# alv-around/mini-stark

Measured on AMD Instinct MI355X. Metric: stark_proofs_per_s, higher is better.
Workload: dtype u64; 1 GPU; Fibonacci AIR, Goldilocks, 2^20 trace rows, blowup 8, 20 security bits (w=3, c=6, rounds=23, ood_queries=1, fri_queries=2); a step = 8 independent proofs in flight per GPU

## Files before the change

### mini-stark_amd/csrc/ctx.hpp

```cpp
#pragma once
#include "../../include/ministark.h"

#include <cstdarg>
#include <cstdio>
#include <cstdlib>
#include <map>
#include <new>
#include <string>
#include <type_traits>
#include <vector>

#include "field.hpp"
#include "merkle.hpp"
#include "ntt.hpp"
#include "poly.hpp"

namespace msctx {

struct DevBuf {
  void* p = nullptr; size_t cap = 0;
  int ensure(size_t bytes) {
    if (bytes <= cap) return 0;
    if (p) msrt::free_dev(p);
    p = nullptr; cap = 0;
// ... 165 lines not shown
    launched();
    if (gx == 0 || gy == 0) return 0;
    if (!prof_on) return msrt::launch_coop<K>(stream, gx, gy, threads, lds, p);
    ProfRec r; r.kid = kid; r.sub = next_sub; r.bytes = next_bytes; r.part = part_depth > 0; next_bytes = 0; next_sub = 0;
    if (msrt::event_create(&r.a) || msrt::event_create(&r.b)) return 1;
    msrt::event_record(r.a, stream);
    int e = msrt::launch_coop<K>(stream, gx, gy, threads, lds, p);
    msrt::event_record(r.b, stream);
    prof_recs.push_back(r);
    return e;
  }
  template <class K> int run(int kid, unsigned gx, unsigned gy, int threads, size_t lds, const typename K::Params& p) {
    launched();
    if (gx == 0 || gy == 0) return 0;
    if (!prof_on) return msrt::launch<K>(stream, gx, gy, threads, lds, p);
    ProfRec r; r.kid = kid; r.sub = next_sub; r.bytes = next_bytes; r.part = part_depth > 0; next_bytes = 0; next_sub = 0;
    if (msrt::event_create(&r.a) || msrt::event_create(&r.b)) return 1;
    msrt::event_record(r.a, stream);
    int e = msrt::launch<K>(stream, gx, gy, threads, lds, p);
    msrt::event_record(r.b, stream);
    prof_recs.push_back(r);
    return e;
  }
  int profile_begin() override { prof_on = true; return 0; }
  int profile_end(char* out, size_t cap) override;

  struct Plan {
    int log_n = 0, log_r0 = 0, log_rho = 0, npass = 0, K[4] = {0, 0, 0, 0}, lo_bits = 0;
    int LC[4] = {msntt::TILE_LOG_C, msntt::TILE_LOG_C, msntt::TILE_LOG_C, msntt::TILE_LOG_C};
    bool v2[4] = {false, false, false, false};
    bool regp[4] = {false, false, false, false};
    DevBuf tw_lo, tw_hi, w_r[4], vtw, w0;
    T n_inv = 0;
  };
  std::map<int, Plan*> plans;
  DevBuf ntt_scratch;
  int ntt_kmax = 9;
  int ntt_v2 = 1, ntt_v2_regpass = 1;
  int ntt_fast = 1;

  int get_plan(int log_n, int log_pad, bool inverse, Plan** out);

  template <bool INV, int K, int TH>
  int launch_fast(const msntt::PassParams<F>& pp, size_t tiles, size_t batch);
  template <class KK> int launch_v2i(const msntt::PassParams<F>& pp, unsigned grid, int nsub, int mode, int k, int lc);
  template <bool INV, int K, int LC, int MODE>
  int launch_v2m(const msntt::PassParams<F>& pp, size_t tiles, size_t batch);
  int ntt_coop_wgs = 512, ntt_share = 1;
  unsigned coop_grid(size_t work_items, int per_cu = 2) const { const size_t g = (size_t)ntt_coop_wgs * per_cu / 2; return (unsigned)(work_items < g ? work_items : g); }
  template <bool INV, int K, int LC>
  int launch_v2(const msntt::PassParams<F>& pp, size_t tiles, size_t batch);
  template <bool INV, int LC>
  int launch_v2k(const msntt::PassParams<F>& pp, size_t tiles, size_t batch);
  template <bool INV, int K>
  int launch_reg(const msntt::PassParams<F>& pp, size_t batch);
  template <bool INV>
  int launch_pass(const msntt::PassParams<F>& pp, size_t tiles, size_t batch, bool v2 = false, bool regp = false);

  int ntt_run(int log_n, bool inverse, const T* src, size_t src_bstride, size_t n_in, T* dst, size_t dst_bstride, size_t batch);
  int scale_pow(const T* src, size_t src_bstride, T* dst, size_t dst_bstride, size_t n, T s, size_t batch);

  void* h_tabs = nullptr; size_t h_tabs_cap = 0;
  int tabs_host(size_t bytes, u8** out);
  DevBuf d_zero; size_t zero_used = 0, zero_cap = 0;
  int zero_alloc(size_t bytes, void** out);

// ... 4 lines not shown
                size_t g_first = 0, u32 run_len = 0, u32 run_stride = 0, const msmerkle::LinColSpec* lin = nullptr, size_t out_g0 = 0);
  template <int EL>
  int tree_build(const T* base, size_t col_stride, size_t row_stride, size_t limb_stride, u32 width, const TreeShape& ts, DevBuf& nodes, const msmerkle::LinColSpec* lin = nullptr);
  u32* host_root() const { return reinterpret_cast<u32*>(reinterpret_cast<u8*>(pinned) + 256); }
  bool root_on_host = false;
  unsigned long long* pending_aux = nullptr; bool aux_on_host = false;
  int inner_levels(u32* nodes, size_t nchildren, size_t ic, bool final_levels = true, u8* rec_out = nullptr);
  int inner_launch(unsigned grid, const msmerkle::InnerHashParams& ip);
  template <int EL>
  int tree_build_sharded(const T* base, size_t col_stride, size_t row_stride, size_t limb_stride, u32 width, TreeShape& ts, DevBuf& nodes, const msmerkle::LinColSpec* lin = nullptr);
  unsigned long long* shard_aux = nullptr;
  int finish_sharded_tree(TreeShape& ts, DevBuf& nodes, size_t Mloc);
  template <int EL>
  int tree_build_sharded_contiguous(const T* base, size_t col_stride, size_t row_stride, size_t limb_stride, u32 width, TreeShape& ts, DevBuf& nodes);
  int read_root(const DevBuf& nodes, const TreeShape& ts, u8* root);

  size_t N = 0, w = 0, L = 0, blowup = 0;
  int npolys = 0; size_t polys_cap = 0;
  struct Lin { std::vector<u64> s; std::vector<int> idx; };
  std::vector<Lin> poly_lin;
  std::vector<char> poly_mat; int lazy_lin = 1;
  void expand(int i, T scale, std::map<int, T>& acc) const {
    const Lin& li = poly_lin[i];
    if (li.idx.empty()) { auto it = acc.find(i); if (it == acc.end()) acc[i] = scale; else it->second = F::add(it->second, scale); return; }
    for (size_t t = 0; t < li.idx.size(); t++) expand(li.idx[t], F::mul(scale, F::from_u64(li.s[t] % F::P)), acc);
  }
  int materialize(int i);
  bool have_trace = false, have_polys = false, have_lde = false, have_validity = false;
  DevBuf d_trace[2], d_polys, d_coef, d_lde, d_trace_nodes, d_lde_nodes, d_io, d_partials, d_small;
  TreeShape trace_ts, lde_ts;
  size_t lde_c = 0;

  struct Round { DevBuf poly, cw, nodes; size_t cap = 0, ncoef = 0, D = 0; TreeShape ts; size_t m = 0;
                 bool dist = false, local_store = false; size_t S = 0; };
  size_t shard_gather_chunk = 0;
  int shard_dist = 1;
  int proof_root_only = 0;
  const T* lpoly(const Round* r) const { return r->local_store ? r->poly.template as<T>() : r->poly.template as<T>() + (size_t)sh_rank * r->S; }
  size_t lstride(const Round* r) const { return r->local_store ? r->S : r->cap; }
  size_t lcount(const Round* r, size_t n) const { const size_t lo = (size_t)sh_rank * r->S; return n <= lo ? 0 : (n - lo < r->S ? n - lo : r->S); }
  size_t dist_chunk(size_t D) const {
    if (!sh_on || !shard_dist || !fri_blowup || !shardable(D / 2)) return 0;
    const size_t den = fri_blowup * (size_t)sh_world;
    if (D % den) return 0;
    const size_t S = D / den;
    return (S >= 2 && !(S & 1)) ? S : 0;
  }
  DevBuf d_carry, d_lq, d_pack, d_fullpoly;
  std::vector<Round*> rounds; size_t nrounds_done = 0, fri_rounds = 0, fri_blowup = 0;
  bool have_deep = false; XE cur_z; XE cur_B[2];
  DevBuf d_folded, d_sh, d_blob, d_tabs, d_targets, d_idx, d_deg, d_ovf;
  size_t blob_size = 0;

  int ensure_polys(size_t count);

  int init(int dev, u32 flags);
  ~Ctx() {
    for (auto& kv : plans) { kv.second->tw_lo.release(); kv.second->tw_hi.release(); kv.second->vtw.release(); kv.second->w0.release(); for (auto& b : kv.second->w_r) b.release(); delete kv.second; }
    drop_rccl();
    if (sdma_pending) msrt::Sdma::get().wait(sdma_sig, -1.0);
    else if (copy_pending) msrt::event_sync(ev_copy);
    if (up.pending) msrt::Sdma::get().wait(sdma_up_sig, -1.0);
    if (sdma_state == 1) { msrt::Sdma::get().signal_destroy(sdma_sig); msrt::Sdma::get().signal_destroy(sdma_up_sig); }
    for (msrt::Event* e : ev_hash) msrt::event_destroy(e);
    for (msrt::Event* e : ev_xchg) msrt::event_destroy(e);
    if (comm_stream) msrt::stream_destroy(comm_stream);
    if (side_stream) { msrt::sync(side_stream); msrt::stream_destroy(side_stream); }
// ... 154 lines not shown
```

### mini-stark_amd/csrc/field.hpp

```cpp
#pragma once
#include "rt.hpp"

typedef uint64_t u64;
typedef uint32_t u32;
typedef uint8_t u8;

struct GL {
  typedef u64 T;
  static constexpr int ID = 0;
  static constexpr u64 P = 0xFFFFFFFF00000001ULL;
  static constexpr u64 EPS = 0xFFFFFFFFULL;
  static constexpr u64 GENERATOR = 7;
  static constexpr int TWO_ADICITY = 32;
  static constexpr int EXT = 2;
  static constexpr u64 NR2 = 7;
  static constexpr int MAX_DIGITS = 20;
  static MS_HD u32 hi(u64 x) { return (u32)(x >> 32); }
  static MS_HD u32 lo(u64 x) { return (u32)x; }
  static MS_HD u64 mk(u32 l, u32 h) { return ((u64)h << 32) | l; }
  static MS_HD T add(T a, T b) {
    const T s = a + b;
    const T t = s - P;
    return (s < a || s >= P) ? t : s;
  }
  static MS_HD T sub(T a, T b) {
    T d = a - b;
    if (a < b) d -= EPS;
    return d;
  }
  static MS_HD T neg(T a) { return a ? P - a : 0; }
  static MS_HD T reduce128(u64 lo_, u64 hi_) {
    const u64 hi_hi = hi_ >> 32, hi_lo = hi_ & EPS;
    u64 t0 = lo_ - hi_hi;
    t0 -= (lo_ < hi_hi) ? EPS : 0;
    const u64 t1 = (hi_lo << 32) - hi_lo;
    const u64 r = t0 + t1;
    const u64 r2 = r + EPS;
    return (r < t1 || r >= P) ? r2 : r;
  }
  static MS_HD T mul(T a, T b) {
    const u32 a0 = (u32)a, a1 = (u32)(a >> 32), b0 = (u32)b, b1 = (u32)(b >> 32);
    const u64 p00 = (u64)a0 * b0;
    const u64 p01 = (u64)a0 * b1 + (p00 >> 32);
    const u64 p10 = (u64)a1 * b0 + (u32)p01;
    const u64 p11 = (u64)a1 * b1 + (p01 >> 32) + (p10 >> 32);
    return reduce128((p10 << 32) | (u32)p00, p11);
  }
  static MS_HD T from_u64(u64 v) { return v; }
  static MS_HD u64 to_u64(T v) { return v; }
  static MS_HD T to_tw(T w) { return w; }
  static MS_HD T tw_of(T w) { return w; }
  static MS_HD T mul_tw(T a, T w_tab) { return mul(a, w_tab); }
  static MS_HD T from_tw(T w_tab) { return w_tab; }
};

struct GLT : GL {
  static MS_HD u64 sel(u32 m, u64 t, u64 s) { return mk(ms_bitop3<0xCA>(m, lo(t), lo(s)), ms_bitop3<0xCA>(m, hi(t), hi(s))); }
  static MS_HD T add(T a, T b) {
    const u64 s = a + b, t = s + EPS;
    const u32 c1 = ms_bitop3<0xD4>(hi(a), hi(b), hi(s));
    const u32 m = ms_sar31(ms_bitop3<0xF4>(c1, hi(s), hi(t)));
    return sel(m, t, s);
  }
  static MS_HD T sub(T a, T b) {
    const u64 d = a - b;
    const u32 bo = ms_bitop3<0x8E>(hi(a), hi(b), hi(d));
    return d + ms_pin64(mk(bo >> 31, ms_sar31(bo)));
  }
  static MS_HD T fold_small(u64 A, u32 h) {
    const u64 r = (u64)h * 0xFFFFFFFFu + A, t = r + EPS;
    return sel(ms_sar31(ms_bitop3<0x74>(hi(A), hi(r), hi(t))), t, r);
  }
  static MS_HD T reduce128(u64 lo_, u64 hi_) {
    const u32 h0 = lo(hi_), h1 = hi(hi_);
    const u64 A = lo_ - h1;
    const u32 b1 = ms_bitop3<0x0C>(hi(lo_), hi(A), 0u);
    const u64 U = (u64)h0 * 0xFFFFFFFFu;
    const u64 r = A + U, t = r + EPS;
    const u32 c1 = ms_bitop3<0xD4>(hi(A), hi(U), hi(r));
    const u32 c2 = ms_bitop3<0x30>(hi(r), hi(t), 0u);
// ... 267 lines not shown
```

### mini-stark_amd/csrc/fri_commit.cpp

```cpp
#include "ctx.hpp"
#include "fri_tail.hpp"

namespace msctx {

template <class F>
int Ctx<F>::round_commit(Round* r, size_t ncoef_in, int nonzero_limbs, const Round* prev, const XE* alpha) {
  if (ctz64(r->D) > F::TWO_ADICITY) return fail(MS_ERR_SHAPE, "FRI domain larger than the field's two-adicity");
  RQ(tree_shape(r->D, 2, 2, &r->ts));
  r->m = 0;
  {
    const bool shard_next = shardable(r->D / 2);
    bool z_outside_base = false;
    for (int l = 1; l < E; l++) z_outside_base = z_outside_base || cur_z.c[l] != 0;
    if (prev && fri_pointwise && z_outside_base && prev->D == 2 * r->D && prev->ts.sharded == shard_next) {
      Plan* pl;
      RQ(get_plan(ctz64(prev->D), 0, false, &pl));
      const size_t W = (size_t)sh_world;
      const size_t m_out = shard_next ? r->D / (2 * W) : r->D;
      const size_t local = shard_next ? 2 * m_out : r->D;
      if (shard_next) r->m = m_out;
      if (r->cw.ensure(local * E * sizeof(T))) return fail(MS_ERR_NOMEM, "codeword");
      const size_t total = m_out * (shard_next ? 2 : 1);
      const XE c = e_add<F, E>(cur_B[0], e_mul<F>(cur_B[1], *alpha));
      auto fold_launch = [&](auto* kernel) {
        typedef typename std::remove_pointer<decltype(kernel)>::type FK;
        typename FK::Params fp;
        fp.src = prev->cw.template as<T>(); fp.src_limb_stride = shard_next ? 2 * prev->m : prev->D;
        fp.dst = r->cw.template as<T>(); fp.dst_limb_stride = local;
        fp.m_out = m_out; fp.log_m = (u32)ctz64(m_out); fp.groups = shard_next ? 2 : 1; fp.shard_W = shard_next ? (u32)W : 0; fp.shard_k = (u32)sh_rank;
        fp.tw_lo = pl->tw_lo.template as<T>(); fp.tw_hi = pl->tw_hi.template as<T>(); fp.lo_bits = (u32)pl->lo_bits; fp.log_D = (u32)ctz64(prev->D);
        fp.alpha = *alpha;
        fp.c2 = e_add<F, E>(c, c);
        fp.z = cur_z;
        fp.inv2 = f_inv<F>(F::from_u64(2));
        return run<FK>(K_FOLD, grid1(total, FK::THREADS * FK::ITEMS), 1, FK::THREADS, 0, fp);
      };
      next_bytes = (double)total * E * sizeof(T) * 3;
      { PartScopeIf part(this, shard_next); CK(total <= fold_small_max ? fold_launch((mspoly::FriFoldEvalKernel<F, E, 1>*)nullptr) : fold_launch((mspoly::FriFoldEvalKernel<F, E, 8>*)nullptr)); }
      if (shard_next) RQ((tree_build_sharded<E>(r->cw.template as<T>(), m_out, 1, 2 * m_out, 2, r->ts, r->nodes)));
      else RQ((tree_build<E>(r->cw.template as<T>(), 0, 1, r->D, 1, r->ts, r->nodes)));
      return 0;
    }
  }
  RQ(join_side());
  if (shardable(r->D / 2)) {
    const size_t m = r->D / (2 * (size_t)sh_world);
    r->m = m;
    if (r->cw.ensure(2 * m * E * sizeof(T))) return fail(MS_ERR_NOMEM, "codeword");
    const T* coef = r->poly.template as<T>(); size_t coef_stride = r->cap;
    if (r->local_store) {
      const size_t full = r->S * (size_t)sh_world;
      if (d_fullpoly.ensure(full * E * sizeof(T))) return fail(MS_ERR_NOMEM, "gathered polynomial");
      if (ncoef_in) RQ(gather_poly(lpoly(r), r->S, ncoef_in, d_fullpoly.as<T>(), full));
      coef = d_fullpoly.as<T>(); coef_stride = full;
    }
    { PartScope part(this); RQ(coset_eval(coef, coef_stride, ncoef_in, ctz64(r->D), F::from_u64(1), 2, r->cw.template as<T>(), 2 * m, (size_t)nonzero_limbs)); }
    if (nonzero_limbs < E) CK(msrt::memset_dev(r->cw.template as<T>() + (size_t)nonzero_limbs * 2 * m, 0, (size_t)(E - nonzero_limbs) * 2 * m * sizeof(T), stream));
    RQ((tree_build_sharded<E>(r->cw.template as<T>(), m, 1, 2 * m, 2, r->ts, r->nodes)));
    return 0;
  }
  if (r->cw.ensure(r->D * E * sizeof(T))) return fail(MS_ERR_NOMEM, "codeword");
  RQ(ntt_run(ctz64(r->D), false, r->poly.template as<T>(), r->cap, ncoef_in, r->cw.template as<T>(), r->D, (size_t)nonzero_limbs));
  if (nonzero_limbs < E) CK(msrt::memset_dev(r->cw.template as<T>() + (size_t)nonzero_limbs * r->D, 0, (size_t)(E - nonzero_limbs) * r->D * sizeof(T), stream));
  RQ((tree_build<E>(r->cw.template as<T>(), 0, 1, r->D, 1, r->ts, r->nodes)));
  return 0;
}

template <class F>
int Ctx<F>::degree_launch(const T* poly, size_t limb_stride, size_t n, unsigned long long** dres_out) {
  void* zr;
  RQ(zero_alloc(8, &zr));
  unsigned long long* dres = reinterpret_cast<unsigned long long*>(zr);
  if (n) {
    typename mspoly::DegreeKernel<F, E>::Params dp{poly, limb_stride, n, dres, 0};
    CK(run<mspoly::DegreeKernel<F, E>>(K_DEGREE, grid1(n, mspoly::THREADS), 1, mspoly::THREADS, 0, dp));
  }
  *dres_out = dres;
  return 0;
}

template <class F>
int Ctx<F>::read_degree_and_root(const T* poly, size_t limb_stride, size_t n, Round* r, size_t* ncoef, u8* root) {
  unsigned long long* dres = nullptr;
  RQ(degree_launch(poly, limb_stride, n, &dres));
  const bool on_host = r && root_on_host;
  CK(msrt::d2h(pinned, dres, 8, stream));
  if (r && !on_host) CK(msrt::d2h(reinterpret_cast<u8*>(pinned) + 64, r->nodes.template as<u8>() + (r->ts.local_nodes - 1) * 32, 32, stream));
  CK(msrt::sync(stream));
  *ncoef = (size_t)(*reinterpret_cast<unsigned long long*>(pinned));
  if (r && root) memcpy(root, on_host ? reinterpret_cast<const u8*>(host_root()) : reinterpret_cast<const u8*>(pinned) + 64, 32);
  return 0;
}

template <class F>
int Ctx<F>::fri_begin(size_t blowup_, size_t nrounds, u8* root0) {
  if (!have_validity) return fail(MS_ERR_STATE, "fri_begin before mix");
// ... 170 lines not shown
    CK(run<CKn>(K_SUFFIX_HORNER, 1, 1, CKn::THREADS, 0, cp));
    if (mj) for (int l = pl.nl - 1; l >= 0; l--) RQ(sh_launch_inline(pl.fin[l], 1));
    nq_coef = m - 1;
  }
  nr->S = Sn;
  if (next_dist) { nr->dist = true; nr->local_store = true; }
  else {
    if (nr->poly.ensure(nr->cap * E * sizeof(T))) return fail(MS_ERR_NOMEM, "fold");
    if (nq_coef) RQ(gather_poly(lq, Sn, nq_coef, nr->poly.template as<T>(), nr->cap));
    nr->S = 0;
  }
  *nq_coef_out = nq_coef;
  return 0;
}

template <class F>
int Ctx<F>::fri_tail_round(Round* pr, Round* nr, const XE& a, bool* done) {
  if (digest == MS_DIGEST_KECCAK256) return fri_tail_round_t<msmerkle::Keccak256Kernels>(pr, nr, a, done);
  if (digest == MS_DIGEST_SHA3_256) return fri_tail_round_t<msmerkle::Sha3_256Kernels>(pr, nr, a, done);
  if (digest == MS_DIGEST_BLAKE3) return fri_tail_round_t<msmerkle::Blake3Kernels>(pr, nr, a, done);
  return digest == MS_DIGEST_BLAKE2S256 ? fri_tail_round_t<msmerkle::Blake2sKernels>(pr, nr, a, done) : fri_tail_round_t<msmerkle::Sha256Kernels>(pr, nr, a, done);
}
template <class F> template <class DG>
int Ctx<F>::fri_tail_round_t(Round* pr, Round* nr, const XE& a, bool* done) {
  *done = false;
  const size_t n = pr->ncoef, m = (n + 1) / 2, Dn = nr->D, M = Dn / 2;
  bool z_outside_base = false;
  for (int l = 1; l < E; l++) z_outside_base = z_outside_base || cur_z.c[l] != 0;
  if (!fri_tail_max || pr->D > fri_tail_max || pr->dist || pr->ts.sharded || shardable(M) || !fri_pointwise || !z_outside_base || m > (size_t)mspoly::SH_BS || M < 1) return 0;
  typedef msfri::FriTailKernel<F, E, DG> TK;
  if (M > (size_t)TK::WG_GROUPS << TK::TreeK::MAX_LEVELS) return 0;
  if (ctz64(Dn) > F::TWO_ADICITY) return fail(MS_ERR_SHAPE, "FRI domain larger than the field's two-adicity");
  RQ(tree_shape(Dn, 2, 2, &nr->ts));
  nr->m = 0;
  if (nr->poly.ensure(nr->cap * E * sizeof(T)) || d_folded.ensure((m + 1) * E * sizeof(T)) || nr->cw.ensure(Dn * E * sizeof(T)) || nr->nodes.ensure(nr->ts.nodes * 32) ||
      d_sh.ensure(sh_scratch_elems(m) * sizeof(T)))
    return fail(MS_ERR_NOMEM, "fused FRI round");
  Plan* pl;
  RQ(get_plan(ctz64(pr->D), 0, false, &pl));
  typename TK::Params tp;
  memset(&tp, 0, sizeof tp);
  tp.do_coef = m >= 2 ? 1 : 0;
  tp.fold = typename TK::FoldK::Params{pr->poly.template as<T>(), pr->cap, n, d_folded.as<T>(), m, a, nullptr};
  if (tp.do_coef) {
    SHPlan sp = sh_plan(d_folded.as<T>(), m, 0, 1, m, cur_z, nr->poly.template as<T>(), false, nr->cap, 0, 1, nullptr, d_sh.as<T>());
    if (sp.nl != 1) return fail(MS_ERR_STATE, "fused FRI round: scan of more than one block");
    tp.scan.jobs = nullptr; tp.scan.inline_job = sp.fin[0]; tp.scan.final_mode = 1;
  }
  unsigned long long* dres = d_deg.as<unsigned long long>();
  tp.deg = typename TK::DegK::Params{nr->poly.template as<T>(), nr->cap, m >= 2 ? m - 1 : 0, dres, 0};
  const size_t per = M < (size_t)TK::WG_GROUPS ? M : (size_t)TK::WG_GROUPS, G = M / per;
  tp.G = (u32)G;
  const XE c = e_add<F, E>(cur_B[0], e_mul<F>(cur_B[1], a));
  tp.eval.src = pr->cw.template as<T>(); tp.eval.src_limb_stride = pr->D; tp.eval.dst = nr->cw.template as<T>(); tp.eval.dst_limb_stride = Dn;
  tp.eval.m_out = Dn; tp.eval.log_m = (u32)ctz64(Dn); tp.eval.groups = 1; tp.eval.shard_W = 0; tp.eval.shard_k = 0;
  tp.eval.tw_lo = pl->tw_lo.template as<T>(); tp.eval.tw_hi = pl->tw_hi.template as<T>(); tp.eval.lo_bits = (u32)pl->lo_bits; tp.eval.log_D = (u32)ctz64(pr->D);
  tp.eval.alpha = a; tp.eval.c2 = e_add<F, E>(c, c); tp.eval.z = cur_z; tp.eval.inv2 = f_inv<F>(F::from_u64(2));
  tp.leaf.base = nr->cw.template as<T>(); tp.leaf.col_stride = 0; tp.leaf.row_stride = 1; tp.leaf.limb_stride = Dn; tp.leaf.width = 1; tp.leaf.lpn = 2;
  tp.leaf.zero_as_empty = zae; tp.leaf.ngroups = M; tp.leaf.nodes = nr->nodes.template as<u32>();
  u32 nl = 0; while (((size_t)1 << nl) < per) nl++;
  tp.sub.nodes = nr->nodes.template as<u32>(); tp.sub.child_off = 0; tp.sub.nchildren = M; tp.sub.ic = 2; tp.sub.nlevels = nl;
  u32 tl = 0; while (((size_t)1 << tl) < G) tl++;
  tp.top.nodes = nr->nodes.template as<u32>(); tp.top.child_off = 2 * M - 2 * G; tp.top.nchildren = G; tp.top.ic = 2; tp.top.nlevels = tl;
  tp.top.host_root = host_root(); tp.top.aux_src = dres; tp.top.aux_dst = reinterpret_cast<unsigned long long*>(pinned); tp.top.flag = arm_flag();
  tp.root_index = nr->ts.nodes - 1;
  tp.done = reinterpret_cast<u32*>(d_deg.as<u8>() + 128);
  next_bytes = (double)Dn * E * sizeof(T) * 3 + (double)M * 96;
// ... 115 lines not shown
```

### mini-stark_amd/csrc/ntt_plan.cpp

```cpp
#include "ctx.hpp"

namespace msctx {

template <class F>
int Ctx<F>::get_plan(int log_n, int log_pad, bool inverse, Plan** out) {
  int key = (log_n * 4 + log_pad) * 2 + (inverse ? 1 : 0);
  auto it = plans.find(key);
  if (it != plans.end()) { *out = it->second; return 0; }
  if (log_n > F::TWO_ADICITY) return fail(MS_ERR_SHAPE, "domain larger than the field's two-adicity");
  Plan* pl = new Plan();
  pl->log_n = log_n;
  const int v2_lc = (F::ID == 0) ? 3 : 4;
  bool use_v2 = false;
  if (ntt_v2 >= 1 && log_n >= 14 && log_n > msntt::MAX_LOG_R && (log_pad == 0 || log_pad == 3)) {
    const int m = log_n - log_pad, P = (m + 9) / 10;
    const int kb = (ntt_v2_regpass == 2) ? 7 : 10;
    if (ntt_v2_regpass && m - 2 * kb >= 1 && m - 2 * kb <= 5) {
      use_v2 = true;
      pl->log_rho = 0; pl->log_r0 = log_pad; pl->npass = 3;
      pl->K[0] = kb; pl->K[1] = kb; pl->K[2] = m - 2 * kb;
      pl->LC[0] = log_pad ? 3 : v2_lc; pl->LC[1] = v2_lc; pl->LC[2] = 0;
      pl->v2[0] = pl->v2[1] = true; pl->regp[2] = true;
    } else if (P <= 2 && m / P >= 7) {
      use_v2 = true;
      pl->log_rho = 0; pl->log_r0 = log_pad; pl->npass = P;
      for (int i = 0; i < P; i++) {
        pl->K[i] = m / P + (i < m % P ? 1 : 0); pl->LC[i] = (i == 0 && log_pad) ? 3 : v2_lc; pl->v2[i] = true;
      }
    }
  }
  if (use_v2) {}
  else if (log_n <= msntt::MAX_LOG_R) { pl->npass = 1; pl->K[0] = log_n; }
  else {
    int best_rho = 0, bestP = 1 << 20;
    for (int lr = 0; lr <= (log_pad ? msntt::MAX_LOG_RHO : 0); lr++) {
      const int m = log_n - log_pad - lr;
      if (m < 2) break;
      int P = (m + ntt_kmax - 1) / ntt_kmax;
      if (P < 2 && log_pad == 0) P = 2;
      if (P < 1) P = 1;
      if (P < bestP) { bestP = P; best_rho = lr; }
    }
    if (ntt_fast && bestP > 1 && (log_pad == 0 || (log_n >= 22 && log_n <= 24))) {
      best_rho = 0; log_pad = 0;
      bestP = (log_n + ntt_kmax - 1) / ntt_kmax; if (bestP < 2) bestP = 2;
    }
    pl->log_rho = best_rho; pl->log_r0 = log_pad + best_rho;
    const int m = log_n - pl->log_r0, P = bestP;
    pl->npass = P;
    for (int i = 0; i < P; i++) pl->K[i] = m / P + (i < m % P ? 1 : 0);
  }
  const int log_r0 = pl->log_r0;
  T wn = f_root_of_unity<F>(log_n);
  if (inverse) wn = f_inv<F>(wn);
  const size_t n = (size_t)1 << log_n;
  pl->n_inv = f_inv<F>(F::from_u64(n % F::P));
  pl->lo_bits = (log_n + 1) / 2;
  const size_t nlo = (size_t)1 << pl->lo_bits, nhi = (size_t)1 << (log_n - pl->lo_bits);
  std::vector<T> lo(nlo), hi(nhi);
  T x = F::from_u64(1);
  for (size_t j = 0; j < nlo; j++) { lo[j] = F::to_tw(x); x = F::mul(x, wn); }
  T wh = x;
  x = F::from_u64(1);
  for (size_t j = 0; j < nhi; j++) { hi[j] = F::to_tw(x); x = F::mul(x, wh); }
  if (pl->tw_lo.ensure(nlo * sizeof(T)) || pl->tw_hi.ensure(nhi * sizeof(T))) { delete pl; return fail(MS_ERR_NOMEM, "twiddle tables"); }
  CK(msrt::h2d(pl->tw_lo.p, lo.data(), nlo * sizeof(T), stream));
  CK(msrt::h2d(pl->tw_hi.p, hi.data(), nhi * sizeof(T), stream));
  CK(msrt::sync(stream));
  for (int i = 0; i < pl->npass; i++) {
    const size_t r = (size_t)1 << pl->K[i];
    T wr = f_root_of_unity<F>(pl->K[i]);
    if (inverse) wr = f_inv<F>(wr);
    std::vector<T> tab(r);
    x = F::from_u64(1);
    for (size_t j = 0; j < r; j++) { tab[j] = F::to_tw(x); x = F::mul(x, wr); }
    if (pl->w_r[i].ensure(r * sizeof(T))) { delete pl; return fail(MS_ERR_NOMEM, "w_r table"); }
    CK(msrt::h2d(pl->w_r[i].p, tab.data(), r * sizeof(T), stream));
    CK(msrt::sync(stream));
  }
  if (pl->log_r0) {
    const size_t cnt = (size_t)1 << log_r0;
    T wv = f_root_of_unity<F>(log_r0);
    if (inverse) wv = f_inv<F>(wv);
    std::vector<T> tab(cnt);
    x = F::from_u64(1);
    for (size_t j = 0; j < cnt; j++) { tab[j] = F::to_tw(x); x = F::mul(x, wv); }
    if (pl->w0.ensure(cnt * sizeof(T))) { delete pl; return fail(MS_ERR_NOMEM, "w0 table"); }
// ... 247 lines not shown
```

### mini-stark_amd/csrc/poly.hpp

```cpp
#pragma once
#include "field.hpp"
#include "ntt.hpp"

namespace mspoly {

constexpr int THREADS = 256;

template <class F> struct TransposeInKernel {
  typedef typename F::T T;
  static constexpr int THREADS = mspoly::THREADS;
  struct Params { const u64* src; T* dst; size_t N, w, dst_stride; T rinv; int mont;  u32* bad; };
  static MS_HD int nphases(const Params&) { return 1; }
  static MS_DEV void phase(int, const Params& p, int bx, int, int tid, int nthreads, unsigned char*) {
    const size_t f = (size_t)bx * nthreads + tid;
    if (f >= p.N * p.w) return;
    const size_t row = f / p.w, col = f - row * p.w;
    const u64 raw = p.src[f];
    const bool oob = raw >= F::P;
    if (oob && p.bad) *p.bad = 1;
    T v = F::from_u64(oob ? 0 : raw);
    if (p.mont) v = F::mul(v, p.rinv);
    p.dst[col * p.dst_stride + row] = v;
  }
};
// ... 439 lines not shown
        const size_t ia = t * 2 * p.m_out + i, ib = ia + p.m_out;
        const size_t r = p.shard_W ? 2 * ((size_t)p.shard_k + (size_t)p.shard_W * i) + t : i;
        X a, b;
#pragma unroll
        for (int l = 0; l < E; l++) { a.c[l] = p.src[(size_t)l * p.src_limb_stride + ia]; b.c[l] = p.src[(size_t)l * p.src_limb_stride + ib]; }
        const X s = e_add<F, E>(a, b), d = e_sub<F, E>(a, b);
        const T xinv = w_tab(p, (Dm + 1 - r) & Dm);
        X u;
#pragma unroll
        for (int l = 0; l < E; l++) u.c[l] = F::mul_tw(p.alpha.c[l], xinv);
        const X num = e_sub<F, E>(e_add<F, E>(s, e_mul<F>(u, d)), p.c2);
        const T y = F::from_tw(w_tab(p, (2 * r) & Dm));
        X C;
        inv_parts(p, F::sub(y, p.z.c[0]), &C, &nrm[it]);
        tt[it] = e_mul<F>(num, C);
      }
      pre[it] = run;
      run = F::mul(run, nrm[it]);
    }
    T inv = F::mul(fold_base_inv<F>(run), p.inv2);
#pragma unroll
    for (int it = ITEMS - 1; it >= 0; it--) {
      const size_t j = j0 + (size_t)it * nthreads;
      const T ni = F::mul(inv, pre[it]);
      inv = F::mul(inv, nrm[it]);
      if (j < total) {
#pragma unroll
        for (int l = 0; l < E; l++) p.dst[(size_t)l * p.dst_limb_stride + j] = F::mul(tt[it].c[l], ni);
      }
    }
  }
};

template <class F, int E> struct DegreeKernel {
  typedef typename F::T T;
  static constexpr int THREADS = mspoly::THREADS;
  struct Params { const T* src; size_t limb_stride, n; unsigned long long* result; size_t idx0; };
  static MS_HD int nphases(const Params&) { return 1; }
  static MS_DEV void phase(int, const Params& p, int bx, int, int tid, int nthreads, unsigned char*) {
    const size_t r = (size_t)bx * nthreads + tid;
    if (r >= p.n) return;
    const size_t j = p.n - 1 - r;
    if ((unsigned long long)(p.idx0 + j + 1) <= *reinterpret_cast<volatile unsigned long long*>(p.result)) return;
    bool nz = false, nz_next = false;
    for (int l = 0; l < E; l++) nz = nz || (p.src[(size_t)l * p.limb_stride + j] != 0);
    if (nz && j + 1 < p.n) for (int l = 0; l < E; l++) nz_next = nz_next || (p.src[(size_t)l * p.limb_stride + j + 1] != 0);
    if (nz && !nz_next) msrt::atomic_max_u64(p.result, (unsigned long long)(p.idx0 + j + 1));
  }
};
template <class F, int E> struct FindJob {
  const typename F::T* src; size_t limb_stride, n;
  const typename F::T* targets ; int nt; unsigned long long* result;
  u32 map_g, map_W, map_k; size_t map_m;
};
template <class F, int E> struct FindFirstKernel {
  typedef typename F::T T;
  static constexpr int THREADS = mspoly::THREADS;
  struct Params { const FindJob<F, E>* jobs; FindJob<F, E> inline_job; };
  static MS_HD int nphases(const Params&) { return 1; }
  static MS_DEV void phase(int, const Params& pp, int bx, int by, int tid, int nthreads, unsigned char*) {
    const FindJob<F, E>& p = pp.jobs ? pp.jobs[by] : pp.inline_job;
    const size_t j = (size_t)bx * nthreads + tid;
    if (j >= p.n) return;
    T v[E];
    for (int l = 0; l < E; l++) v[l] = p.src[(size_t)l * p.limb_stride + j];
    for (int t = 0; t < p.nt; t++) {
// ... 177 lines not shown
      const T root = p.ex_roots[k];
#pragma unroll
      for (int it = 0; it < ITEMS; it++) acc[it] = F::mul(acc[it], F::sub(x[it], root));
    }
#pragma unroll
    for (int it = 0; it < ITEMS; it++) {
      const size_t i = i0 + (size_t)it * THREADS;
      if (i < p.L) p.out[i] = F::mul(acc[it], p.den_inv[i & (size_t)(p.blowup - 1)]);
    }
  }
};

template <int S> struct ArithShift { template <class A> static MS_DEV u64 run(u64 x, int s) { return s == S ? msntt::gl_mul_pow2<S, A>(x) : ArithShift<S - 1>::template run<A>(x, s); } };
template <> struct ArithShift<0> { template <class A> static MS_DEV u64 run(u64 x, int) { return x; } };
template <class F, class A> struct ArithKernel {
  typedef typename F::T T;
  static constexpr int THREADS = 256;
  struct Params { const u64* a; const u64* b; u64* out; size_t n; int op; };
  static MS_HD int nphases(const Params&) { return 1; }
  static MS_DEV void phase(int, const Params& p, int bx, int, int tid, int, unsigned char*) {
    const size_t i = (size_t)bx * THREADS + tid;
    if (i >= p.n) return;
    const T a = F::from_u64(p.a[i]), b = F::from_u64(p.b[i]);
    T r = 0;
    if (p.op == 0) r = A::add(a, b);
    else if (p.op == 1) r = A::sub(a, b);
    else if (p.op == 2) r = A::mul(a, b);
    else if (p.op == 3) r = A::mul_tw(a, F::to_tw(b));
    if constexpr (F::ID == 0) {
      if (p.op == 4) r = A::mul_x32(a);
      else if (p.op == 5) r = A::mul_x64(a);
      else if (p.op == 6) r = ArithShift<95>::template run<A>(a, (int)(p.b[i] % 96));
      else if (p.op == 7) r = A::fold_small(a, (u32)p.b[i] & 0x7FFFFFFFu);
    }
    p.out[i] = F::to_u64(r);
  }
};
}
```

### mini-stark_amd/csrc/session.cpp

```cpp
#include "ctx.hpp"

namespace msctx {

template <class F>
int Ctx<F>::profile_end(char* out, size_t cap) {
  static const char* names[K_COUNT] = {"ntt_pass", "scale_pow", "leaf_hash", "inner_hash", "transpose_in", "io_copy", "lincomb", "mix", "eval", "eval_reduce",
                                       "fold", "suffix_horner", "degree", "find_first", "merkle_path", "query_points", "fri_tail", "mix_terms"};
  msrt::sync(stream);
  double ms[K_COUNT] = {0}, by[K_COUNT] = {0}, ms_part = 0, ms_repl = 0, repl_by[K_COUNT] = {0}; unsigned long long cnt[K_COUNT] = {0};
  std::map<int, double> sub_ms, sub_by; std::map<int, unsigned long long> sub_cnt;
  for (auto& r : prof_recs) {
    float t = 0.f; msrt::event_elapsed_ms(&t, r.a, r.b);
    ms[r.kid] += t; by[r.kid] += r.bytes; cnt[r.kid]++;
    if (r.part) ms_part += t; else { ms_repl += t; repl_by[r.kid] += t; }
    if (r.kid == K_NTT_PASS) { sub_ms[r.sub] += t; sub_by[r.sub] += r.bytes; sub_cnt[r.sub]++; }
    msrt::event_destroy(r.a); msrt::event_destroy(r.b);
  }
  prof_recs.clear(); prof_on = false;
  std::string j = "{";
  for (int k = 0; k < K_COUNT; k++) {
    char buf[256];
    snprintf(buf, sizeof buf, "%s\"%s\": {\"launches\": %llu, \"ms\": %.6f, \"alg_bytes\": %.0f}", k ? ", " : "", names[k], cnt[k], ms[k], by[k]);
    j += buf;
  }
// ... 189 lines not shown
  for (int t = 0; t < k; t++) if (idx[t] < 0 || idx[t] >= npolys || s[t] >= F::P) return fail(MS_ERR_ARG, "lincomb index/scalar out of range");
  RQ(ensure_polys(npolys + 2));
  if (!lazy_lin) RQ(lincomb_into(d_polys.as<T>(), N, N, s, idx, k, npolys, d_polys.as<T>() + (size_t)npolys * N));
  poly_mat.push_back(lazy_lin ? 0 : 1);
  { Lin l; l.s.assign(s, s + k); l.idx.assign(idx, idx + k); poly_lin.push_back(l); }
  npolys++; have_lde = have_validity = false;
  return MS_OK;
}

template <class F>
int Ctx<F>::polys_append(const u64* coeffs, size_t n) {
  if (!have_polys) return fail(MS_ERR_STATE, "append before interpolate");
  if (!coeffs || n > N) return fail(MS_ERR_SHAPE, "constraint polynomial has more than N coefficients (starks.rs:118-119 asserts)");
  if (!canonical(coeffs, n)) return fail(MS_ERR_ARG, "coefficient not canonical");
  RQ(ensure_polys(npolys + 2));
  T* dst = d_polys.as<T>() + (size_t)npolys * N;
  CK(msrt::memset_dev(dst, 0, N * sizeof(T), stream));
  if (n) { RQ(upload_narrow(coeffs, n, dst)); CK(msrt::sync(stream)); }
  poly_mat.push_back(1);
  poly_lin.push_back(Lin());
  npolys++; have_lde = have_validity = false;
  return MS_OK;
}

template <class F>
int Ctx<F>::poly_read(int i, u64* out) {
  if (!have_polys || i < 0 || i >= npolys || !out) return fail(MS_ERR_ARG, "poly_read");
  RQ(materialize(i));
  return download_widen(d_polys.as<T>() + (size_t)i * N, N, 0, 1, out);
}

template <class F>
int Ctx<F>::arith_selftest(int op, const u64* a, const u64* b, u64* out, size_t n) {
  if (!a || !b || !out || op < 0 || op > 7 || (F::ID != 0 && op > 3)) return fail(MS_ERR_ARG, "arith_selftest: bad operation / null argument");
  if (!n) return MS_OK;
  if (!canonical(a, n) || (op < 6 && !canonical(b, n))) return fail(MS_ERR_ARG, "operand not canonical");
  DevBuf d;
  if (d.ensure(3 * n * 8)) return fail(MS_ERR_NOMEM, "arith_selftest");
  typedef typename std::conditional<F::ID == 0, GLM, F>::type A;
  typedef mspoly::ArithKernel<F, A> AK;
  int e = msrt::h2d(d.p, a, n * 8, stream);
  if (!e) e = msrt::h2d(d.as<u64>() + n, b, n * 8, stream);
  if (!e) e = msrt::sync(stream);
  typename AK::Params ap{d.as<u64>(), d.as<u64>() + n, d.as<u64>() + 2 * n, n, op};
  if (!e) e = run<AK>(K_IO, grid1(n, AK::THREADS), 1, AK::THREADS, 0, ap);
  if (!e) e = msrt::d2h(out, d.as<u64>() + 2 * n, n * 8, stream);
  if (!e) e = msrt::sync(stream);
  d.release();
  return e ? fail_rt(e, "arith_selftest") : MS_OK;
}

#define MS_INSTANTIATE(FF) \
  template int Ctx<FF>::profile_end(char* out, size_t cap); \
  template int Ctx<FF>::tabs_host(size_t bytes, u8** out); \
  template int Ctx<FF>::zero_alloc(size_t bytes, void** out); \
  template int Ctx<FF>::materialize(int i); \
  template int Ctx<FF>::ensure_polys(size_t count); \
  template int Ctx<FF>::init(int dev, u32 flags); \
  template int Ctx<FF>::upload_narrow(const u64* host, size_t n, Ctx<FF>::T* dst); \
  template int Ctx<FF>::download_widen(const Ctx<FF>::T* src, size_t n, size_t limb_stride, u32 e, u64* host); \
  template int Ctx<FF>::transpose_in(const u64* src, Ctx<FF>::T* dst, size_t rows, size_t cols, Ctx<FF>::T rinv, int mont, u32* bad); \
  template int Ctx<FF>::trace_commit(const u64* trace, bool on_device, size_t N_, size_t w_, size_t lpn, u8* root); \
  template int Ctx<FF>::interpolate(); \
  template int Ctx<FF>::polys_lincomb(const u64* s, const int* idx, int k); \
  template int Ctx<FF>::polys_append(const u64* coeffs, size_t n); \
  template int Ctx<FF>::poly_read(int i, u64* out); \
  template int Ctx<FF>::arith_selftest(int op, const u64* a, const u64* b, u64* out, size_t n);
// ... 6 lines not shown
```

Measured before the change: 276.6 proofs/s.

## Add workgroup-batched FRI fold kernel with octet twiddle layout and base-field sources

Replaces the per-item FRI fold-eval kernel for large rounds with a workgroup kernel. It batches the DEEP denominator inversions across the whole workgroup using one shared-memory prefix-product inversion. When the domain allows, it groups 8 related points per thread so that twiddles become multiplications by powers of two (shift-based mul_pow2) instead of table loads and full multiplies. It also tracks whether the previous codeword has only a base-field limb, so the fold reads one limb instead of E. This adds complexity and new correctness risk in the octet index and sign mapping, plus extra barriers and cooperative launches.

```diff
diff --git a/mini-stark_amd/csrc/ctx.hpp b/mini-stark_amd/csrc/ctx.hpp
--- a/mini-stark_amd/csrc/ctx.hpp
+++ b/mini-stark_amd/csrc/ctx.hpp
@@ -221,6 +221,7 @@
     bool regp[4] = {false, false, false, false};
     DevBuf tw_lo, tw_hi, w_r[4], vtw, w0;
     T n_inv = 0;
+    T root = 0;
   };
   std::map<int, Plan*> plans;
   DevBuf ntt_scratch;
@@ -291,7 +292,8 @@
   size_t lde_c = 0;
 
   struct Round { DevBuf poly, cw, nodes; size_t cap = 0, ncoef = 0, D = 0; TreeShape ts; size_t m = 0;
-                 bool dist = false, local_store = false; size_t S = 0; };
+                 bool dist = false, local_store = false; size_t S = 0;
+                 bool base_cw = false;  };
   size_t shard_gather_chunk = 0;
   int shard_dist = 1;
   int proof_root_only = 0;
diff --git a/mini-stark_amd/csrc/field.hpp b/mini-stark_amd/csrc/field.hpp
--- a/mini-stark_amd/csrc/field.hpp
+++ b/mini-stark_amd/csrc/field.hpp
@@ -46,6 +46,22 @@
     const u64 p11 = (u64)a1 * b1 + (p01 >> 32) + (p10 >> 32);
     return reduce128((p10 << 32) | (u32)p00, p11);
   }
+  template <int S> static MS_HD T mul_pow2(T x) {
+    static_assert(S >= 0 && S < 96, "shift out of range");
+    if constexpr (S == 0) return x;
+    else {
+      constexpr int b = S & 31, w = S >> 5;
+      const u64 l = x << b;
+      u32 t2 = 0;
+      if constexpr (b != 0) t2 = (u32)(x >> (64 - b));
+      if constexpr (w == 0) return reduce128(l, t2);
+      else if constexpr (w == 1) return reduce128((u64)lo(l) << 32, mk(hi(l), t2));
+      else return sub(((u64)lo(l) << 32) - lo(l), mk(hi(l), t2));
+    }
+  }
+  static MS_HD T mul_2p24(T x) { return mul_pow2<24>(x); }
+  static MS_HD T mul_2p48(T x) { return mul_pow2<48>(x); }
+  static MS_HD T mul_2p72(T x) { return mul_pow2<72>(x); }
   static MS_HD T from_u64(u64 v) { return v; }
   static MS_HD u64 to_u64(T v) { return v; }
   static MS_HD T to_tw(T w) { return w; }
diff --git a/mini-stark_amd/csrc/fri_commit.cpp b/mini-stark_amd/csrc/fri_commit.cpp
--- a/mini-stark_amd/csrc/fri_commit.cpp
+++ b/mini-stark_amd/csrc/fri_commit.cpp
@@ -8,6 +8,7 @@
   if (ctz64(r->D) > F::TWO_ADICITY) return fail(MS_ERR_SHAPE, "FRI domain larger than the field's two-adicity");
   RQ(tree_shape(r->D, 2, 2, &r->ts));
   r->m = 0;
+  r->base_cw = false;
   {
     const bool shard_next = shardable(r->D / 2);
     bool z_outside_base = false;
@@ -22,9 +23,7 @@
       if (r->cw.ensure(local * E * sizeof(T))) return fail(MS_ERR_NOMEM, "codeword");
       const size_t total = m_out * (shard_next ? 2 : 1);
       const XE c = e_add<F, E>(cur_B[0], e_mul<F>(cur_B[1], *alpha));
-      auto fold_launch = [&](auto* kernel) {
-        typedef typename std::remove_pointer<decltype(kernel)>::type FK;
-        typename FK::Params fp;
+      auto fold_params = [&](auto& fp) {
         fp.src = prev->cw.template as<T>(); fp.src_limb_stride = shard_next ? 2 * prev->m : prev->D;
         fp.dst = r->cw.template as<T>(); fp.dst_limb_stride = local;
         fp.m_out = m_out; fp.log_m = (u32)ctz64(m_out); fp.groups = shard_next ? 2 : 1; fp.shard_W = shard_next ? (u32)W : 0; fp.shard_k = (u32)sh_rank;
@@ -33,10 +32,42 @@
         fp.c2 = e_add<F, E>(c, c);
         fp.z = cur_z;
         fp.inv2 = f_inv<F>(F::from_u64(2));
+      };
+      auto fold_launch = [&](auto* kernel) {
+        typedef typename std::remove_pointer<decltype(kernel)>::type FK;
+        typename FK::Params fp;
+        fold_params(fp);
         return run<FK>(K_FOLD, grid1(total, FK::THREADS * FK::ITEMS), 1, FK::THREADS, 0, fp);
       };
-      next_bytes = (double)total * E * sizeof(T) * 3;
-      { PartScopeIf part(this, shard_next); CK(total <= fold_small_max ? fold_launch((mspoly::FriFoldEvalKernel<F, E, 1>*)nullptr) : fold_launch((mspoly::FriFoldEvalKernel<F, E, 8>*)nullptr)); }
+      u32 oct_q[8] = {0, 0, 0, 0, 0, 0, 0, 0}, oct_neg = 0;
+      bool oct = false;
+      if constexpr (F::ID == 0) {
+        if (!shard_next && m_out >= 8 && (m_out & (m_out - 1)) == 0) {
+          const T w16 = f_pow<F>(pl->root, (u64)(prev->D / 16));
+          for (u32 mm = 1; mm < 16 && !oct; mm += 2) {
+            if (f_pow<F>(F::from_u64((u64)1 << 12), mm) != w16) continue;
+            u32 minv = 1; while ((mm * minv) % 16 != 1) minv += 2;
+            for (u32 k = 0; k < 8; k++) { const u32 e = (k * minv) % 16; oct_q[k] = e % 8; if ((e >= 8) != (k > 0)) oct_neg |= 1u << k; }
+            oct = true;
+          }
+        }
+      }
+      auto wg_launch = [&](auto* kernel) {
+        typedef typename std::remove_pointer<decltype(kernel)>::type FK;
+        typename FK::Params wp;
+        fold_params(wp.f);
+        for (int k = 0; k < 8; k++) wp.oct_q[k] = oct_q[k];
+        wp.oct_neg = oct_neg;
+        return run_coop<FK>(K_FOLD, grid1(FK::grid_items(wp), FK::THREADS), FK::THREADS, FK::lds_bytes(), wp);
+      };
+      const bool src1 = prev->base_cw;
+      next_bytes = (double)total * (E + 2 * (src1 ? 1 : E)) * sizeof(T);
+      { PartScopeIf part(this, shard_next);
+        if (total <= fold_small_max) CK(fold_launch((mspoly::FriFoldEvalKernel<F, E, 1>*)nullptr));
+        else if constexpr (F::ID == 0) {
+          if (oct) CK(src1 ? wg_launch((mspoly::FriFoldWgKernel<F, E, 1, true>*)nullptr) : wg_launch((mspoly::FriFoldWgKernel<F, E, E, true>*)nullptr));
+          else CK(src1 ? wg_launch((mspoly::FriFoldWgKernel<F, E, 1, false>*)nullptr) : wg_launch((mspoly::FriFoldWgKernel<F, E, E, false>*)nullptr));
+        } else CK(src1 ? wg_launch((mspoly::FriFoldWgKernel<F, E, 1, false>*)nullptr) : wg_launch((mspoly::FriFoldWgKernel<F, E, E, false>*)nullptr)); }
       if (shard_next) RQ((tree_build_sharded<E>(r->cw.template as<T>(), m_out, 1, 2 * m_out, 2, r->ts, r->nodes)));
       else RQ((tree_build<E>(r->cw.template as<T>(), 0, 1, r->D, 1, r->ts, r->nodes)));
       return 0;
@@ -56,12 +87,14 @@
     }
     { PartScope part(this); RQ(coset_eval(coef, coef_stride, ncoef_in, ctz64(r->D), F::from_u64(1), 2, r->cw.template as<T>(), 2 * m, (size_t)nonzero_limbs)); }
     if (nonzero_limbs < E) CK(msrt::memset_dev(r->cw.template as<T>() + (size_t)nonzero_limbs * 2 * m, 0, (size_t)(E - nonzero_limbs) * 2 * m * sizeof(T), stream));
+    r->base_cw = nonzero_limbs == 1;
     RQ((tree_build_sharded<E>(r->cw.template as<T>(), m, 1, 2 * m, 2, r->ts, r->nodes)));
     return 0;
   }
   if (r->cw.ensure(r->D * E * sizeof(T))) return fail(MS_ERR_NOMEM, "codeword");
   RQ(ntt_run(ctz64(r->D), false, r->poly.template as<T>(), r->cap, ncoef_in, r->cw.template as<T>(), r->D, (size_t)nonzero_limbs));
   if (nonzero_limbs < E) CK(msrt::memset_dev(r->cw.template as<T>() + (size_t)nonzero_limbs * r->D, 0, (size_t)(E - nonzero_limbs) * r->D * sizeof(T), stream));
+  r->base_cw = nonzero_limbs == 1;
   RQ((tree_build<E>(r->cw.template as<T>(), 0, 1, r->D, 1, r->ts, r->nodes)));
   return 0;
 }
@@ -298,7 +331,7 @@
   if (M > (size_t)TK::WG_GROUPS << TK::TreeK::MAX_LEVELS) return 0;
   if (ctz64(Dn) > F::TWO_ADICITY) return fail(MS_ERR_SHAPE, "FRI domain larger than the field's two-adicity");
   RQ(tree_shape(Dn, 2, 2, &nr->ts));
-  nr->m = 0;
+  nr->m = 0; nr->base_cw = false;
   if (nr->poly.ensure(nr->cap * E * sizeof(T)) || d_folded.ensure((m + 1) * E * sizeof(T)) || nr->cw.ensure(Dn * E * sizeof(T)) || nr->nodes.ensure(nr->ts.nodes * 32) ||
       d_sh.ensure(sh_scratch_elems(m) * sizeof(T)))
     return fail(MS_ERR_NOMEM, "fused FRI round");
diff --git a/mini-stark_amd/csrc/ntt_plan.cpp b/mini-stark_amd/csrc/ntt_plan.cpp
--- a/mini-stark_amd/csrc/ntt_plan.cpp
+++ b/mini-stark_amd/csrc/ntt_plan.cpp
@@ -53,6 +53,7 @@
   const int log_r0 = pl->log_r0;
   T wn = f_root_of_unity<F>(log_n);
   if (inverse) wn = f_inv<F>(wn);
+  pl->root = wn;
   const size_t n = (size_t)1 << log_n;
   pl->n_inv = f_inv<F>(F::from_u64(n % F::P));
   pl->lo_bits = (log_n + 1) / 2;
diff --git a/mini-stark_amd/csrc/poly.hpp b/mini-stark_amd/csrc/poly.hpp
--- a/mini-stark_amd/csrc/poly.hpp
+++ b/mini-stark_amd/csrc/poly.hpp
@@ -495,6 +495,155 @@
   }
 };
 
+template <class F, int E, int SRC_LIMBS_ = E, bool OCT_ = false> struct FriFoldWgKernel {
+  typedef typename F::T T;
+  typedef Ext<F, E> X;
+  typedef FriFoldEvalKernel<F, E, 1> Lat;
+  static_assert(E == 2 || E == 4, "quadratic or quartic tower");
+  static_assert(SRC_LIMBS_ == 1 || SRC_LIMBS_ == E, "base-field or full source");
+  static_assert(!OCT_ || F::ID == 0, "the octet layout needs Goldilocks' roots of unity");
+  static constexpr int THREADS = mspoly::THREADS, ITEMS = 8, NW = THREADS / 64, SRC_LIMBS = SRC_LIMBS_;
+  static constexpr bool OCT = OCT_;
+  struct Params {
+    typename Lat::Params f;
+    u32 oct_q[8];
+    u32 oct_neg;
+  };
+  static MS_HD size_t lds_bytes() { return (size_t)THREADS * sizeof(T); }
+  static MS_HD size_t grid_items(const Params& p) { return OCT ? p.f.m_out / 8 : (p.f.m_out * p.f.groups + ITEMS - 1) / ITEMS; }
+  struct ZPre { T nz; Ext<F, 2> zb, K; };
+  static MS_DEV ZPre z_pre(const X& z) {
+    ZPre zp;
+    const T nr = F::from_u64(F::NR2);
+    zp.nz = 0; zp.zb = e_zero<F, 2>(); zp.K = e_zero<F, 2>();
+    if constexpr (E == 2) zp.nz = F::mul(nr, F::mul(z.c[1], z.c[1]));
+    else { zp.zb.c[0] = z.c[2]; zp.zb.c[1] = z.c[3]; zp.K = e_mul_nr4<F>(e_mul<F>(zp.zb, zp.zb)); }
+    return zp;
+  }
+  static MS_DEV void inv_parts(const X& z, const ZPre& zp, T yd, X* C, T* n) {
+    if constexpr (E == 2) {
+      C->c[0] = yd; C->c[1] = z.c[1];
+      *n = F::sub(F::mul(yd, yd), zp.nz);
+    } else {
+      const T nr = F::from_u64(F::NR2);
+      Ext<F, 2> A;
+      A.c[0] = yd; A.c[1] = F::neg(z.c[1]);
+      const Ext<F, 2> M = e_sub<F, 2>(e_mul<F>(A, A), zp.K);
+      Ext<F, 2> Mc; Mc.c[0] = M.c[0]; Mc.c[1] = F::neg(M.c[1]);
+      *n = F::sub(F::mul(M.c[0], M.c[0]), F::mul(nr, F::mul(M.c[1], M.c[1])));
+      const Ext<F, 2> c0 = e_mul<F>(A, Mc), c1 = e_mul<F>(zp.zb, Mc);
+      C->c[0] = c0.c[0]; C->c[1] = c0.c[1]; C->c[2] = c1.c[0]; C->c[3] = c1.c[1];
+    }
+  }
+  template <int S> static MS_DEV void item(const typename Lat::Params& p, const ZPre& zp, size_t ia, size_t ib, const X& u, T y, X* tt, T* nrm) {
+    T a[SRC_LIMBS], b[SRC_LIMBS];
+#pragma unroll
+    for (int l = 0; l < SRC_LIMBS; l++) { a[l] = p.src[(size_t)l * p.src_limb_stride + ia]; b[l] = p.src[(size_t)l * p.src_limb_stride + ib]; }
+    X num;
+    if constexpr (SRC_LIMBS == E) {
+      X s, d;
+#pragma unroll
+      for (int l = 0; l < E; l++) {
+        s.c[l] = F::add(a[l], b[l]); d.c[l] = F::sub(a[l], b[l]);
+        if constexpr (S != 0) d.c[l] = F::template mul_pow2<S>(d.c[l]);
+      }
+      num = e_sub<F, E>(e_add<F, E>(s, e_mul<F>(u, d)), p.c2);
+    } else {
+      const T s0 = F::add(a[0], b[0]);
+      T d0 = F::sub(a[0], b[0]);
+      if constexpr (S != 0) d0 = F::template mul_pow2<S>(d0);
+      num.c[0] = F::sub(F::add(s0, F::mul(u.c[0], d0)), p.c2.c[0]);
+#pragma unroll
+      for (int l = 1; l < E; l++) num.c[l] = F::sub(F::mul(u.c[l], d0), p.c2.c[l]);
+    }
+    X C;
+    inv_parts(p.z, zp, F::sub(y, p.z.c[0]), &C, nrm);
+    *tt = e_mul<F>(num, C);
+  }
+  template <int K> static MS_DEV void oct_items(const Params& pp, const ZPre& zp, bool act, size_t i0, size_t Q, const X& u0, T y0, X* tt, T* nrm, T* pre, T* prod) {
+    if constexpr (K < ITEMS) {
+      tt[K] = e_zero<F, E>(); nrm[K] = F::from_u64(1);
+      if (act) {
+        const size_t i = i0 + (size_t)pp.oct_q[K] * Q;
+        const bool ng = (pp.oct_neg >> K) & 1u;
+        T y = F::template mul_pow2<24 * (K & 3)>(y0);
+        if constexpr (K >= 4) y = F::neg(y);
+        item<(K ? 96 - 12 * K : 0)>(pp.f, zp, ng ? i + pp.f.m_out : i, ng ? i : i + pp.f.m_out, u0, y, &tt[K], &nrm[K]);
+      }
+      pre[K] = *prod;
+      *prod = F::mul(*prod, nrm[K]);
+      oct_items<K + 1>(pp, zp, act, i0, Q, u0, y0, tt, nrm, pre, prod);
+    }
+  }
+  static MS_DEV void run(const Params& pp, int bx, int, int, int tid, unsigned char* lds) {
+    const typename Lat::Params& p = pp.f;
+    const size_t total = p.m_out * p.groups, Dm = ((size_t)1 << p.log_D) - 1;
+    const ZPre zp = z_pre(p.z);
+    X tt[ITEMS]; T nrm[ITEMS], pre[ITEMS];
+    T prod = F::from_u64(1);
+    const size_t Q = p.m_out / 8;
+    size_t j0;
+    if constexpr (OCT) {
+      j0 = (size_t)bx * THREADS + tid;
+      const bool act = j0 < Q;
+      X u0 = e_zero<F, E>(); T y0 = 0;
+      if (act) {
+        const T xinv = Lat::w_tab(p, (Dm + 1 - j0) & Dm);
+#pragma unroll
+        for (int l = 0; l < E; l++) u0.c[l] = F::mul_tw(p.alpha.c[l], xinv);
+        y0 = F::from_tw(Lat::w_tab(p, (2 * j0) & Dm));
+      }
+      oct_items<0>(pp, zp, act, j0, Q, u0, y0, tt, nrm, pre, &prod);
+    } else {
+      j0 = (size_t)bx * ((size_t)THREADS * ITEMS) + tid;
+#pragma unroll
+      for (int it = 0; it < ITEMS; it++) {
+        const size_t j = j0 + (size_t)it * THREADS;
+        tt[it] = e_zero<F, E>(); nrm[it] = F::from_u64(1);
+        if (j < total) {
+          const size_t t = j >> p.log_m, i = j & (p.m_out - 1);
+          const size_t ia = t * 2 * p.m_out + i;
+          const size_t r = p.shard_W ? 2 * ((size_t)p.shard_k + (size_t)p.shard_W * i) + t : i;
+          const T xinv = Lat::w_tab(p, (Dm + 1 - r) & Dm);
+          X u;
+#pragma unroll
+          for (int l = 0; l < E; l++) u.c[l] = F::mul_tw(p.alpha.c[l], xinv);
+          item<0>(p, zp, ia, ia + p.m_out, u, F::from_tw(Lat::w_tab(p, (2 * r) & Dm)), &tt[it], &nrm[it]);
+        }
+        pre[it] = prod;
+        prod = F::mul(prod, nrm[it]);
+      }
+    }
+    T* sp = reinterpret_cast<T*>(lds);
+    sp[tid] = prod;
+    msrt::wg_barrier();
+    if (tid < 64) {
+      const int ln = tid;
+      T a[NW], ap[NW];
+      T acc = F::from_u64(1);
+#pragma unroll
+      for (int w = 0; w < NW; w++) { a[w] = sp[ln + 64 * w]; ap[w] = acc; acc = w ? F::mul(acc, a[w]) : a[w]; }
+      T iv = F::mul(fold_base_inv<F>(acc), p.inv2);
+#pragma unroll
+      for (int w = NW - 1; w >= 0; w--) { sp[ln + 64 * w] = w ? F::mul(iv, ap[w]) : iv; if (w) iv = F::mul(iv, a[w]); }
+    }
+    msrt::wg_barrier();
+    T inv = sp[tid];
+#pragma unroll
+    for (int it = ITEMS - 1; it >= 0; it--) {
+      size_t j; bool in;
+      if constexpr (OCT) { in = j0 < Q; j = j0 + (size_t)pp.oct_q[it] * Q; }
+      else { j = j0 + (size_t)it * THREADS; in = j < total; }
+      const T ni = F::mul(inv, pre[it]);
+      inv = F::mul(inv, nrm[it]);
+      if (in) {
+#pragma unroll
+        for (int l = 0; l < E; l++) p.dst[(size_t)l * p.dst_limb_stride + j] = F::mul(tt[it].c[l], ni);
+      }
+    }
+  }
+};
+
 template <class F, int E> struct DegreeKernel {
   typedef typename F::T T;
   static constexpr int THREADS = mspoly::THREADS;
@@ -738,6 +887,21 @@
       else if (p.op == 5) r = A::mul_x64(a);
       else if (p.op == 6) r = ArithShift<95>::template run<A>(a, (int)(p.b[i] % 96));
       else if (p.op == 7) r = A::fold_small(a, (u32)p.b[i] & 0x7FFFFFFFu);
+      else if (p.op == 8) r = GL::mul_2p24(a);
+      else if (p.op == 9) r = GL::mul_2p48(a);
+      else if (p.op == 10) r = GL::mul_2p72(a);
+      else if (p.op == 11) {
+        switch ((int)(p.b[i] & 7)) {
+          case 0: r = a; break;
+          case 1: r = GL::mul_pow2<12>(a); break;
+          case 2: r = GL::mul_pow2<24>(a); break;
+          case 3: r = GL::mul_pow2<36>(a); break;
+          case 4: r = GL::mul_pow2<48>(a); break;
+          case 5: r = GL::mul_pow2<60>(a); break;
+          case 6: r = GL::mul_pow2<72>(a); break;
+          default: r = GL::mul_pow2<84>(a); break;
+        }
+      }
     }
     p.out[i] = F::to_u64(r);
   }
diff --git a/mini-stark_amd/csrc/session.cpp b/mini-stark_amd/csrc/session.cpp
--- a/mini-stark_amd/csrc/session.cpp
+++ b/mini-stark_amd/csrc/session.cpp
@@ -245,7 +245,7 @@
 
 template <class F>
 int Ctx<F>::arith_selftest(int op, const u64* a, const u64* b, u64* out, size_t n) {
-  if (!a || !b || !out || op < 0 || op > 7 || (F::ID != 0 && op > 3)) return fail(MS_ERR_ARG, "arith_selftest: bad operation / null argument");
+  if (!a || !b || !out || op < 0 || op > 11 || (F::ID != 0 && op > 3)) return fail(MS_ERR_ARG, "arith_selftest: bad operation / null argument");
   if (!n) return MS_OK;
   if (!canonical(a, n) || (op < 6 && !canonical(b, n))) return fail(MS_ERR_ARG, "operand not canonical");
   DevBuf d;
```

Result: faster. 280.7 proofs/s (median of 6 runs) (+1.5%).
